# haoyu94/RoITr

Measured on AMD Instinct MI355X. Metric: point-cloud pairs/s, higher is better.
Workload: dtype f32; 1 GPU; 3DMatch-sized synthetic pairs: 5000 pts/cloud src+tgt, fp32, 3DMatch test settings (P=256 patches x 64 pts, 100 Sinkhorn iterations), full RIGA_v2 forward; n_points=5000, weights=closed-form, variant 'selective' (roitr_amd/weights.py); normals: field, cloud=uniform, correspondences_found=66241567

## Files before the change

include/roitr_engine.h:

```cpp
#ifndef ROITR_ENGINE_H
#define ROITR_ENGINE_H

#include <stddef.h>

#ifdef __cplusplus
extern "C" {
#endif

#ifndef ROITR_POINTOPS_H
typedef struct ihipStream_t* roitr_stream_t;
#endif

typedef struct RoitrGemm {
    int M, N, K;
    const float* A; const float* A2; int lda; const int* a_idx; int a_limit;
    const float* W; int ldw; const int* w_idx; int w_limit;
    const float* bias; float alpha; int relu;
    float* C; int ldc;
    int batch; long sA, sW, sC, sBias, sAidx, sWidx;
    const int* seg_off; int seg_a0, seg_w0;
    const float* ln_gamma; const float* ln_beta; const float* ln_res; const int* ln_res_idx; const float* ln_post;
    int ln_relu; float ln_eps;
    int bf16;
    const float* A_cat; int lda_cat; int k_cat;
// ... 177 lines not shown
int roitr_optimal_transport(const RoitrOT* a, roitr_stream_t stream);
int roitr_ot_stats(int enable, unsigned long long* out);

typedef struct RoitrFine {
    int pairs, num_corr, limit, k, mutual;
    float conf;
    const int* n_corr; const float* ot; const int* row_masks; const int* col_masks;
    const float* row_pts; const float* col_pts; const float* global_scores;
    unsigned char* flags; int* counts; int* offsets; int* n_out;
    float* out_row_pts; float* out_col_pts; float* out_scores; int* out_patch;
    long out_cap;
    const int* pair_off; int slots;
    int* pair_starts;
} RoitrFine;
int roitr_fine_matching(const RoitrFine* a, roitr_stream_t stream);

int roitr_build_padded_clouds(int pairs, int n_points, const float* pts, const int* pt_offset, const float* rot,
                              const float* trans, float* out_pts, int* out_offset, roitr_stream_t stream);
int roitr_node_occlusion_score(int n_nodes, int limit, const int* cloud_of_node, const int* pt_offset, const int* knn_idx,
                               const int* knn_mask, const int* node_masks, const float* d2_padded, float overlap_thres,
                               float* out, roitr_stream_t stream);
typedef struct RoitrNodeCorr {
    int pairs, limit, max_nodes;
    float pos_radius;
    const float* nodes; const int* node_offset; const int* node_masks;
    const float* points; const int* pt_offset; const int* knn_idx; const int* knn_mask;
    const float* rot; const float* trans;
    float* overlap; long mat_stride;
    int* out_idx; float* out_overlap; int* out_count;
    int n_nodes; float* nodes_t; float* radius;
// ... 73 lines not shown
```

roitr_amd/csrc/engine.cpp:

```cpp
#include <hip/hip_runtime.h>
#include <math.h>
#include <stdio.h>
#include <string.h>

#include <functional>
#include <map>
#include <string>
#include <vector>

#include "common.h"
#include "prof.h"
#include "roitr_engine.h"
#include "roitr_pointops.h"

extern "C" int roitr_build_pfold(int H, int heads, const float* wpe, const float* bpe, float* pfold, hipStream_t stream);

#define CHK(x)                    \
    do {                          \
        int s__ = (x);            \
        if (s__ != 0) return s__; \
    } while (0)

namespace {

// ... 1451 lines not shown
        c.tgt_corr = tgt_corr; c.src_corr = src_corr; c.corr_scores = cscore; c.n_corr = n_corr;
        c.xy = cxy; c.xy_stride = xystride; c.xy_ld = V.nmax[3];
        if (E.cfg.adaptive_coarse) CHK(roitr_adaptive_matching(&c, E.cfg.num_corr, 0.75f, st));
        else CHK(roitr_coarse_matching(&c, st));
    }
    if (compact) CHK(roitr_patch_offsets(B, n_corr, (int)NP, pair_off, st));
    const int* live_patches = compact ? pair_off + B : nullptr;
    {
        RoitrPatch pg; memset(&pg, 0, sizeof(pg));
        pg.pairs = B; pg.num_corr = P_; pg.limit = LIM; pg.n_corr = n_corr; pg.tgt_corr = tgt_corr; pg.src_corr = src_corr;
        pg.node_offset = D.off[3]; pg.pt_offset = D.off[0]; pg.knn_idx = kidx; pg.knn_mask = kmask; pg.points = pts_out;
        pg.tgt_rows = trows; pg.src_rows = srows; pg.tgt_masks = tmask; pg.src_masks = smask; pg.tgt_pts = tpts; pg.src_pts = spts;
        pg.pair_off = pair_off; pg.slots = compact ? (int)NP : 0;
        CHK(roitr_patch_gather(&pg, st));
    }
    {
        RoitrGemm g; memset(&g, 0, sizeof(g));
        g.M = LIM; g.N = LIM; g.K = C4; g.A = point_feats; g.lda = C4; g.a_idx = trows; g.a_limit = T1; g.W = point_feats; g.ldw = C4;
        g.w_idx = srows; g.w_limit = T1; g.alpha = 1.0f / sqrtf((float)C4); g.C = mscore; g.ldc = LIM; g.batch = (int)NP;
        g.sC = (long)LIM * LIM; g.sAidx = LIM; g.sWidx = LIM;
        g.batch_live = live_patches;
        if (E.cfg.operand_dtype == 1) {
            unsigned short* pf_h = A.get<unsigned short>((size_t)T1 * C4);
            if (A.fail) { roitr_set_error("arena exhausted (matching)", __FILE__, __LINE__); return ROITR_ERR_ARG; }
            RoitrGemm gh = g;
            gh.A = reinterpret_cast<const float*>(pf_h); gh.W = reinterpret_cast<const float*>(pf_h); gh.bf16 = ROITR_BF16_W | ROITR_BF16_A;
            if (roitr_gemm_bf16_supported(&gh)) {
                CHK(roitr_f32_to_bf16((long)T1 * C4, point_feats, pf_h, st));
                g = gh;
            }
        }
        CHK(roitr_gemm(&g, st));
    }
    {
        RoitrOT o; memset(&o, 0, sizeof(o));
        o.pairs = B; o.num_corr = P_; o.limit = LIM; o.num_iter = 100; o.n_corr = n_corr; o.scores = mscore; o.row_masks = tmask;
        o.col_masks = smask; o.alpha = E.ot_alpha; o.out = ot;
        o.pair_off = pair_off; o.slots = compact ? (int)NP : 0;
        CHK(roitr_optimal_transport(&o, st));
    }
    {
        RoitrFine fm; memset(&fm, 0, sizeof(fm));
        fm.pairs = B; fm.num_corr = P_; fm.limit = LIM; fm.k = E.cfg.fine_topk; fm.mutual = E.cfg.fine_mutual; fm.conf = E.cfg.fine_conf;
        fm.n_corr = n_corr; fm.ot = ot; fm.row_masks = tmask; fm.col_masks = smask; fm.row_pts = tpts; fm.col_pts = spts;
        fm.global_scores = E.cfg.fine_use_global_score ? cscore : nullptr;
        fm.flags = flags; fm.counts = counts; fm.offsets = offsets; fm.n_out = n_out;
        fm.out_row_pts = o_t; fm.out_col_pts = o_s; fm.out_scores = o_sc; fm.out_patch = io->out_patch; fm.out_cap = (long)cap;
        fm.pair_off = pair_off; fm.slots = compact ? (int)NP : 0; fm.pair_starts = io->pair_starts;
        CHK(roitr_fine_matching(&fm, st));
    }
    roitr_prof_end(ROITR_PROF_PH_MATCH, st);
    roitr_prof_end(ROITR_PROF_PH_FORWARD, st);
    return 0;
}


extern "C" int roitr_engine_forward_graph(void* h, const RoitrForwardIO* io, hipStream_t st)
{
    Engine& E = *(Engine*)h;
    if (!E.finalized) { roitr_set_error("engine not finalized", __FILE__, __LINE__); return ROITR_ERR_ARG; }
    if (!st || roitr_prof_is_enabled() || !E.taps.empty() || !E.injects.empty() || io->pairs <= 0) return roitr_engine_forward(h, io, st);
    std::vector<long> key;
    key.push_back(io->pairs);
// ... 73 lines not shown
```

roitr_amd/csrc/matching.hip:

```cpp
#include "common.h"
#include <cstdio>
#include <cstdlib>
#include "prof.h"
#include "roitr_engine.h"

namespace {

__device__ __forceinline__ float sq_norm3(float x, float y, float z)
{
#pragma clang fp contract(off)
    const float a = x * x, b = y * y, c = z * z;
    return (a + b) + c;
}
__device__ __forceinline__ float square_distance3(float sx, float sy, float sz, float s2, float tx, float ty, float tz, float t2)
{
#pragma clang fp contract(off)
    const float m = sx * tx;
    const float xy = __fmaf_rn(sz, tz, __fmaf_rn(sy, ty, m));
    const float a = -2.0f * xy;
    const float b = a + s2;
    return fmaxf(b + t2, 1e-12f);
}

__global__ __launch_bounds__(256) void p2n_assign_kernel(int n_points, const float* __restrict__ pts, const int* __restrict__ pt_offset,
// ... 381 lines not shown
    OT_TERM(s0, B, KARR, T_, 8); OT_TERM(s1, B, KARR, T_, 9); OT_TERM(s2, B, KARR, T_, 10); OT_TERM(s3, B, KARR, T_, 11);   \
    OT_TERM(s0, B, KARR, T_, 12); OT_TERM(s1, B, KARR, T_, 13); OT_TERM(s2, B, KARR, T_, 14); OT_TERM(s3, B, KARR, T_, 15)
__device__ __forceinline__ float ot_dot64(const float (&KARR)[64], float x, float init, int lane)
{
    const float x1 = __int_as_float(__builtin_amdgcn_ds_bpermute(((lane + 16) & 63) << 2, __float_as_int(x)));
    const float x2 = __int_as_float(__builtin_amdgcn_ds_bpermute(((lane + 32) & 63) << 2, __float_as_int(x)));
    const float x3 = __int_as_float(__builtin_amdgcn_ds_bpermute(((lane + 48) & 63) << 2, __float_as_int(x)));
    float s0 = init, s1 = 0.f, s2 = 0.f, s3 = 0.f;
    asm volatile("s_nop 1" : : "v"(x), "v"(s1), "v"(s2), "v"(s3));
    OT_BLOCK(x, KARR, 0);
    OT_BLOCK(x1, KARR, 1);
    OT_BLOCK(x2, KARR, 2);
    OT_BLOCK(x3, KARR, 3);
    return (s0 + s1) + (s2 + s3);
}
__global__ __launch_bounds__(64) void ot_kernel(RoitrOT a, unsigned long long* stats)
{
    __shared__ float T[64][65];
    __shared__ __attribute__((aligned(16))) float av[64];
    const int patch = blockIdx.x;
    const int lane = threadIdx.x;
    if (a.pair_off ? patch >= a.pair_off[a.pairs] : (patch % a.num_corr) >= a.n_corr[patch / a.num_corr]) return;
    float* out = a.out + (size_t)patch * OTN * OTN;
    const float alpha = *a.alpha;
    const float* sc = a.scores + (size_t)patch * 64 * 64;
    const bool rml = a.row_masks[(size_t)patch * 64 + lane] != 0, cml = a.col_masks[(size_t)patch * 64 + lane] != 0;
    const unsigned long long rbits = __ballot(rml), cbits = __ballot(cml);
    const int nvr = __popcll(rbits), nvc = __popcll(cbits);
    const float norm = -logf((float)nvr + (float)nvc);
#pragma unroll 8
    for (int i = 0; i < 64; ++i) T[i][lane] = sc[i * 64 + lane];
    __syncthreads();
    float KR[64], KC[64];
    float m = rml ? alpha : -1e6f;
    float lo = alpha;
#pragma unroll
    for (int j = 0; j < 64; ++j) {
        const bool ok = rml && ((cbits >> j) & 1);
        const float v = ok ? T[lane][j] : -1e6f;
        KR[j] = v;
        m = fmaxf(m, v);
        lo = ok ? fminf(lo, v) : lo;
    }
    if (__ballot(rml && m - lo > OT_FAST_SPREAD) != 0) {
        if (lane == 0) out[64 * OTN + 64] = __int_as_float(0x7fc00000);
        return;
    }
#pragma unroll
    for (int j = 0; j < 64; ++j) {
        KR[j] = (rml && ((cbits >> j) & 1)) ? expf(KR[j] - m) : 0.f;
        T[lane][j] = KR[j];
    }
    const float krd = rml ? expf(alpha - m) : 0.f;
    const float kdr = cml ? 1.0f : 0.f;
    const float kdd = 1.0f;
    __syncthreads();
    {
        const int R = lane >> 4, c = lane & 15;
#pragma unroll
        for (int t = 0; t < 4; ++t)
#pragma unroll
            for (int n = 0; n < 16; ++n) {
                const int e = ((R + t) & 3) * 16 + ((c - n) & 15);
                KR[t * 16 + n] = T[lane][e];
                KC[t * 16 + n] = T[e][lane];
            }
    }
    const float mu = rml ? expf(norm) : 0.f, nu = cml ? expf(norm) : 0.f;
    const float mu64 = expf(logf((float)nvc) + norm), nu64 = expf(logf((float)nvr) + norm);
    float al = 0.f, a64 = 0.f, bl = cml ? 1.0f : 0.f, b64 = 1.0f;
    for (int it = 0; it < a.num_iter; ++it) {
        const float rs = ot_dot64(KR, bl, krd * b64, lane);
        al = rml ? mu / rs : 0.f;
        a64 = mu64 / (wave_sum(kdr * bl) + kdd * b64);
        const float cs = ot_dot64(KC, al, kdr * a64, lane);
        const float bn = cml ? nu / cs : 0.f;
        const float b64n = nu64 / (wave_sum(krd * al) + kdd * a64);
        const bool same = __ballot(__float_as_int(bn) != __float_as_int(bl)) == 0 && __float_as_int(b64n) == __float_as_int(b64);
        bl = bn; b64 = b64n;
        if (same) { if (stats && lane == 0) atomicAdd(stats + 1, (unsigned long long)(a.num_iter - 1 - it)); break; }
    }
    if (stats && lane == 0) atomicAdd(stats, 1ull);
    {
        const bool bad = (rml && !(al > 0.f && al < INFINITY)) || (cml && !(bl > 0.f && bl < INFINITY)) || !(a64 > 0.f && a64 < INFINITY) ||
                         !(b64 > 0.f && b64 < INFINITY);
        if (__ballot(bad) != 0) {
            if (lane == 0) out[64 * OTN + 64] = __int_as_float(0x7fc00000);
            return;
        }
    }
    __syncthreads();
    const float ul = rml ? logf(al) - m : 0.f, vl = cml ? logf(bl) : 0.f;
    const float u64 = logf(a64) - alpha, v64 = logf(b64);
    av[lane] = ul;
    __syncthreads();
#pragma unroll 8
    for (int i = 0; i < 64; ++i) {
        const float sv = (cml && ((rbits >> i) & 1)) ? sc[i * 64 + lane] : -1e6f;
        out[i * OTN + lane] = sv + av[i] + vl - norm;
    }
    out[64 * OTN + lane] = (cml ? alpha : -1e6f) + u64 + vl - norm;
    out[lane * OTN + 64] = (rml ? alpha : -1e6f) + ul + v64 - norm;
    if (lane == 0) out[64 * OTN + 64] = alpha + u64 + v64 - norm;
}

#define OTL_ROT(X, N_) __int_as_float(__builtin_amdgcn_update_dpp(0, __float_as_int(X), 0x120 + (N_), 0xf, 0xf, false))
#define OTL_LOAD16(XA, SARR, VB, T_)                                                                                         \
    XA[(T_) * 16] = SARR[(T_) * 16] + VB;                                                                                     \
    XA[(T_) * 16 + 1] = SARR[(T_) * 16 + 1] + OTL_ROT(VB, 1);   XA[(T_) * 16 + 2] = SARR[(T_) * 16 + 2] + OTL_ROT(VB, 2);     \
    XA[(T_) * 16 + 3] = SARR[(T_) * 16 + 3] + OTL_ROT(VB, 3);   XA[(T_) * 16 + 4] = SARR[(T_) * 16 + 4] + OTL_ROT(VB, 4);     \
    XA[(T_) * 16 + 5] = SARR[(T_) * 16 + 5] + OTL_ROT(VB, 5);   XA[(T_) * 16 + 6] = SARR[(T_) * 16 + 6] + OTL_ROT(VB, 6);     \
    XA[(T_) * 16 + 7] = SARR[(T_) * 16 + 7] + OTL_ROT(VB, 7);   XA[(T_) * 16 + 8] = SARR[(T_) * 16 + 8] + OTL_ROT(VB, 8);     \
    XA[(T_) * 16 + 9] = SARR[(T_) * 16 + 9] + OTL_ROT(VB, 9);   XA[(T_) * 16 + 10] = SARR[(T_) * 16 + 10] + OTL_ROT(VB, 10); \
    XA[(T_) * 16 + 11] = SARR[(T_) * 16 + 11] + OTL_ROT(VB, 11); XA[(T_) * 16 + 12] = SARR[(T_) * 16 + 12] + OTL_ROT(VB, 12); \
    XA[(T_) * 16 + 13] = SARR[(T_) * 16 + 13] + OTL_ROT(VB, 13); XA[(T_) * 16 + 14] = SARR[(T_) * 16 + 14] + OTL_ROT(VB, 14); \
    XA[(T_) * 16 + 15] = SARR[(T_) * 16 + 15] + OTL_ROT(VB, 15)
__device__ __forceinline__ float ot_lse65(const float (&SARR)[64], float x, float extra, int lane)
{
// ... 9 lines not shown
#pragma unroll
    for (int i = 0; i < 64; ++i) mx = fmaxf(mx, X[i]);
    float s0 = __expf(extra - mx), s1 = 0.f, s2 = 0.f, s3 = 0.f;
#pragma unroll
    for (int i = 0; i < 64; i += 4) {
        s0 += __expf(X[i] - mx); s1 += __expf(X[i + 1] - mx); s2 += __expf(X[i + 2] - mx); s3 += __expf(X[i + 3] - mx);
    }
    return mx + __logf((s0 + s1) + (s2 + s3));
}
__device__ __forceinline__ float ot_lse_wave(float x, float extra)
{
    const float mx = fmaxf(wave_max(x), extra);
    return mx + __logf(wave_sum(__expf(x - mx)) + __expf(extra - mx));
}

__global__ __launch_bounds__(64) void ot_log_kernel(RoitrOT a, unsigned long long* stats)
{
    __shared__ float T[64][65];
    const int patch = blockIdx.x;
    const int lane = threadIdx.x;
    if (a.pair_off ? patch >= a.pair_off[a.pairs] : (patch % a.num_corr) >= a.n_corr[patch / a.num_corr]) return;
    float* out = a.out + (size_t)patch * OTN * OTN;
    {
        const float corner = out[64 * OTN + 64];
        if (corner == corner) return;
    }
    if (stats && lane == 0) atomicAdd(stats + 2, 1ull);
    const float alpha = *a.alpha;
    const float NINF = -1e6f;
    const float* sc = a.scores + (size_t)patch * 64 * 64;
    const bool rml = a.row_masks[(size_t)patch * 64 + lane] != 0, cml = a.col_masks[(size_t)patch * 64 + lane] != 0;
    const unsigned long long rbits = __ballot(rml), cbits = __ballot(cml);
    const int nvr = __popcll(rbits), nvc = __popcll(cbits);
    const float norm = -logf((float)nvr + (float)nvc);
#pragma unroll 8
    for (int i = 0; i < 64; ++i) T[i][lane] = (cml && ((rbits >> i) & 1)) ? sc[i * 64 + lane] : NINF;
// ... 23 lines not shown
        vl = vn;
    }
    __syncthreads();
    T[0][lane] = ul;
    __syncthreads();
#pragma unroll 8
    for (int i = 0; i < 64; ++i) {
        const float sv = (cml && ((rbits >> i) & 1)) ? sc[i * 64 + lane] : NINF;
        out[i * OTN + lane] = sv + T[0][i] + vl - norm;
    }
    out[64 * OTN + lane] = sdr + u64 + vl - norm;
    out[lane * OTN + 64] = srd + ul + v64 - norm;
    if (lane == 0) out[64 * OTN + 64] = alpha + u64 + v64 - norm;
}

__device__ __forceinline__ unsigned long long topk_mask(float v, int k, float conf)
{
    const int lane = threadIdx.x & 63;
    bool sel = false;
    for (int t = 0; t < k; ++t) {
        const float cand = sel ? -1.f : v;
        const float m = wave_max(cand);
        const unsigned long long eq = __ballot(cand == m);
        if (m >= 0.f && lane == __ffsll((long long)eq) - 1) sel = true;
    }
    return __ballot(sel && v > conf);
}

__global__ __launch_bounds__(256) void fine_flag_kernel(RoitrFine a)
{
    __shared__ float E[64][65];
    __shared__ unsigned long long rowm[64], colm[64];
    __shared__ int cnt_s[4];
    const int patch = blockIdx.x;
    const int tid = threadIdx.x, lane = tid & 63, wave = tid >> 6;
    const int L = a.limit;
    unsigned char* fl = a.flags + (size_t)patch * L * L;
    uint4* fl16 = reinterpret_cast<uint4*>(fl) + tid;
    if (a.pair_off ? patch >= a.pair_off[a.pairs] : (patch % a.num_corr) >= a.n_corr[patch / a.num_corr]) {
        if (tid == 0) a.counts[patch] = 0;
        return;
    }
    const float* sc = a.ot + (size_t)patch * (L + 1) * (L + 1);
    for (int e = tid; e < L * L; e += 256) { const int i = e >> 6, j = e & 63; E[i][j] = expf(sc[i * (L + 1) + j]); }
    __syncthreads();
    if (a.k <= 4) {
        if (wave < 2) {
            float bv[4] = {-1.f, -1.f, -1.f, -1.f};
            int bi[4] = {0, 0, 0, 0};
#pragma unroll 8
            for (int j = 0; j < 64; ++j) {
                float x = wave == 0 ? E[lane][j] : E[j][lane];
                int xi = j;
#pragma unroll
                for (int t = 0; t < 4; ++t) {
                    const bool up = x > bv[t];
                    const float tv = bv[t]; const int ti = bi[t];
                    bv[t] = up ? x : tv; bi[t] = up ? xi : ti;
                    x = up ? tv : x; xi = up ? ti : xi;
                }
            }
            unsigned long long m = 0ull;
#pragma unroll
            for (int t = 0; t < 4; ++t)
                if (t < a.k && bv[t] >= 0.f && bv[t] > a.conf) m |= 1ull << bi[t];
            if (wave == 0) rowm[lane] = m; else colm[lane] = m;
        }
    } else {
        for (int r = wave; r < 64; r += 4) {
            const unsigned long long mr = topk_mask(E[r][lane], a.k, a.conf);
            const unsigned long long mc = topk_mask(E[lane][r], a.k, a.conf);
            if (lane == 0) { rowm[r] = mr; colm[r] = mc; }
        }
    }
    __syncthreads();
    const int i = tid >> 2, j0 = (tid & 3) * 16;
    const int* cm = a.col_masks + (size_t)patch * L;
    const bool row_ok = a.row_masks[(size_t)patch * L + i] != 0;
    const unsigned long long rmask = rowm[i];
    unsigned w[4] = {0, 0, 0, 0};
    int local = 0;
#pragma unroll
    for (int jj = 0; jj < 16; ++jj) {
        const int j = j0 + jj;
        const bool rt = (rmask >> j) & 1, ct = (colm[j] >> i) & 1;
        const bool f = (a.mutual ? (rt && ct) : (rt || ct)) && row_ok && cm[j] != 0;
        w[jj >> 2] |= (f ? 1u : 0u) << (8 * (jj & 3));
        local += f ? 1 : 0;
    }
    *fl16 = make_uint4(w[0], w[1], w[2], w[3]);
    local = (int)wave_sum((float)local);
    if (lane == 0) cnt_s[wave] = local;
    __syncthreads();
    if (tid == 0) a.counts[patch] = cnt_s[0] + cnt_s[1] + cnt_s[2] + cnt_s[3];
}

__global__ __launch_bounds__(1024) void fine_scan_kernel(int n, const int* __restrict__ counts, int* __restrict__ offsets, int* __restrict__ n_out,
                                                         long out_cap, int pairs, int num_corr, const int* __restrict__ pair_off,
                                                         int* __restrict__ pair_starts)
{
    __shared__ int wsum[16];
    __shared__ int carry_s;
    const int tid = threadIdx.x, lane = tid & 63, wave = tid >> 6;
    if (tid == 0) carry_s = 0;
    __syncthreads();
    for (int base = 0; base < n; base += 1024) {
        const int i = base + tid;
        const int v = i < n ? counts[i] : 0;
        int incl = v;
// ... 52 lines not shown
    for (int u = 0; u < per; ++u) {
        const int e = tid * per + u;
        if (((fw[u >> 2] >> (8 * (u & 3))) & 1u) && pos < cap) {
            const int i = e / L, j = e % L;
            const float* rp = a.row_pts + ((size_t)patch * L + i) * 3;
            const float* cp = a.col_pts + ((size_t)patch * L + j) * 3;
            a.out_row_pts[(size_t)pos * 3] = rp[0]; a.out_row_pts[(size_t)pos * 3 + 1] = rp[1]; a.out_row_pts[(size_t)pos * 3 + 2] = rp[2];
            a.out_col_pts[(size_t)pos * 3] = cp[0]; a.out_col_pts[(size_t)pos * 3 + 1] = cp[1]; a.out_col_pts[(size_t)pos * 3 + 2] = cp[2];
            a.out_scores[pos] = expf(sc[i * (L + 1) + j]) * g;
            if (a.out_patch) a.out_patch[pos] = patch;
            ++pos;
        }
    }
}

}

extern "C" int roitr_point_to_node_partition(int b, int n_points, int n_nodes, const float* pts, const int* pt_offset,
                                             const float* nodes, const int* node_offset, const int* cloud_of_node, int limit,
                                             int* p2n, float* p2n_dist, int* node_masks, int* knn_idx, int* knn_mask, hipStream_t stream)
{
    if (n_points <= 0 || n_nodes <= 0) return ROITR_OK;
    ROITR_HIP(hipMemsetAsync(node_masks, 0, sizeof(int) * (size_t)n_nodes, stream));
    p2n_assign_kernel<<<div_up(n_points, 256), 256, 0, stream>>>(n_points, pts, pt_offset, nullptr, nodes, node_offset, b, p2n, p2n_dist, node_masks);
    ROITR_LAUNCH_CHECK();
    p2n_topk_kernel<<<n_nodes, 256, 0, stream>>>(pt_offset, node_offset, cloud_of_node, p2n, p2n_dist, limit, knn_idx, knn_mask);
    ROITR_LAUNCH_CHECK();
    return ROITR_OK;
}

// ... 115 lines not shown
    if (a->limit != 64) return ROITR_ERR_UNSUPPORTED;
    const int patches = a->pair_off ? a->slots : a->pairs * a->num_corr;
    if (patches <= 0) {
        ROITR_HIP(hipMemsetAsync(a->n_out, 0, sizeof(int), stream));
        if (a->pair_starts) ROITR_HIP(hipMemsetAsync(a->pair_starts, 0, sizeof(int) * ((size_t)a->pairs + 1), stream));
        return ROITR_OK;
    }
    fine_flag_kernel<<<patches, 256, 0, stream>>>(*a);
    ROITR_LAUNCH_CHECK();
    fine_scan_kernel<<<1, 1024, 0, stream>>>(patches, a->counts, a->offsets, a->n_out, a->out_cap, a->pairs, a->num_corr, a->pair_off, a->pair_starts);
    ROITR_LAUNCH_CHECK();
    fine_emit_kernel<<<patches, 256, 0, stream>>>(*a);
    ROITR_LAUNCH_CHECK();
    return ROITR_OK;
}
```

roitr_amd/ops.py:

```python
import torch

from . import _lib as L


def _i32c(t):
    return t.to(torch.int32).contiguous()


def calc_ppf(points, point_normals, ref_points, ref_normals, group_idx):
    m, k = group_idx.shape
    out = torch.empty((m, k, 4), dtype=torch.float32, device=points.device)
    grp = _i32c(group_idx)
    L.check(L.lib().roitr_calc_ppf(m, k, L.ptr(points.contiguous()), L.ptr(point_normals.contiguous()),
                                   L.ptr(ref_points.contiguous()), L.ptr(ref_normals.contiguous()), L.ptr(grp), L.ptr(out),
                                   L.stream_ptr()), "calc_ppf")
    return out


def calc_ppf_gpu(points, point_normals, patches, patch_normals):
    m, k, _ = patches.shape
    grp = torch.arange(m * k, dtype=torch.int32, device=points.device).view(m, k)
    return calc_ppf(points, point_normals, patches.reshape(-1, 3), patch_normals.reshape(-1, 3), grp)


# ... 90 lines not shown
    offs = torch.zeros(B, dtype=i32, device=dev)
    n_out = torch.zeros(1, dtype=i32, device=dev)
    o_r = torch.zeros((cap, 3), dtype=torch.float32, device=dev)
    o_c = torch.zeros((cap, 3), dtype=torch.float32, device=dev)
    o_s = torch.zeros(cap, dtype=torch.float32, device=dev)
    rm, cm = ref_knn_masks.to(i32).contiguous(), src_knn_masks.to(i32).contiguous()
    rp, cp = ref_knn_points.contiguous().float(), src_knn_points.contiguous().float()
    ms = matching_scores.contiguous().float()
    gs = global_scores.contiguous().float() if global_scores is not None else None
    a = _Fine(1, B, Lm, int(k), int(mutual), float(confidence_threshold), L.ptr(nc), L.ptr(ms), L.ptr(rm), L.ptr(cm), L.ptr(rp),
              L.ptr(cp), L.ptr(gs), L.ptr(flags), L.ptr(counts), L.ptr(offs), L.ptr(n_out), L.ptr(o_r), L.ptr(o_c), L.ptr(o_s), L.ptr(None), cap)
    L.check(L.lib().roitr_fine_matching(ctypes.byref(a), L.stream_ptr()), "fine_matching")
    n = int(n_out.item())
    return o_r[:n], o_c[:n], o_s[:n]


class _Gemm(ctypes.Structure):
    _fields_ = [("M", ctypes.c_int), ("N", ctypes.c_int), ("K", ctypes.c_int), ("A", _P), ("A2", _P), ("lda", ctypes.c_int),
                ("a_idx", _P), ("a_limit", ctypes.c_int), ("W", _P), ("ldw", ctypes.c_int), ("w_idx", _P), ("w_limit", ctypes.c_int),
                ("bias", _P), ("alpha", ctypes.c_float), ("relu", ctypes.c_int), ("C", _P), ("ldc", ctypes.c_int),
                ("batch", ctypes.c_int), ("sA", ctypes.c_long), ("sW", ctypes.c_long), ("sC", ctypes.c_long),
                ("sBias", ctypes.c_long), ("sAidx", ctypes.c_long), ("sWidx", ctypes.c_long), ("seg_off", _P),
                ("seg_a0", ctypes.c_int), ("seg_w0", ctypes.c_int),
                ("ln_gamma", _P), ("ln_beta", _P), ("ln_res", _P), ("ln_res_idx", _P), ("ln_post", _P),
                ("ln_relu", ctypes.c_int), ("ln_eps", ctypes.c_float), ("bf16", ctypes.c_int),
                ("A_cat", _P), ("lda_cat", ctypes.c_int), ("k_cat", ctypes.c_int),
                ("ip_feat", _P), ("ip_idx", _P), ("ip_dist2", _P), ("a_cat_idx", _P), ("batch_live", _P), ("w_piece", ctypes.c_long)]


BF16_W, BF16_A, BF16_C, BF16_X3 = 1, 2, 4, 8
# ... 269 lines not shown
```

Measured before the change: 6336 pairs/s.

## Fuse patch score GEMM, Sinkhorn OT and fine flagging into one kernel

For the fp32 operand path, a single patch_match kernel now computes each patch's 64x64 similarity tile, runs the exp-domain Sinkhorn solve and produces the fine top-k flags, all with the tile kept in shared memory. This avoids writing the score matrix out and reading it back across separate GEMM, OT and flag launches. Patches that fail the fast exp solve are appended to a declined list and handled afterwards by grid-stride log-domain OT and flag kernels. The cost is a heavier per-block kernel with one 64-thread wave per patch, plus an extra atomic-driven fallback path.

```diff
diff --git a/include/roitr_engine.h b/include/roitr_engine.h
--- a/include/roitr_engine.h
+++ b/include/roitr_engine.h
@@ -215,6 +215,7 @@
     int* pair_starts;
 } RoitrFine;
 int roitr_fine_matching(const RoitrFine* a, roitr_stream_t stream);
+int roitr_patch_match(const RoitrGemm* g, const RoitrOT* o, const RoitrFine* f, int* declined, roitr_stream_t stream);
 
 int roitr_build_padded_clouds(int pairs, int n_points, const float* pts, const int* pt_offset, const float* rot,
                               const float* trans, float* out_pts, int* out_offset, roitr_stream_t stream);
diff --git a/roitr_amd/csrc/engine.cpp b/roitr_amd/csrc/engine.cpp
--- a/roitr_amd/csrc/engine.cpp
+++ b/roitr_amd/csrc/engine.cpp
@@ -1489,39 +1489,37 @@
         pg.pair_off = pair_off; pg.slots = compact ? (int)NP : 0;
         CHK(roitr_patch_gather(&pg, st));
     }
-    {
-        RoitrGemm g; memset(&g, 0, sizeof(g));
-        g.M = LIM; g.N = LIM; g.K = C4; g.A = point_feats; g.lda = C4; g.a_idx = trows; g.a_limit = T1; g.W = point_feats; g.ldw = C4;
-        g.w_idx = srows; g.w_limit = T1; g.alpha = 1.0f / sqrtf((float)C4); g.C = mscore; g.ldc = LIM; g.batch = (int)NP;
-        g.sC = (long)LIM * LIM; g.sAidx = LIM; g.sWidx = LIM;
-        g.batch_live = live_patches;
-        if (E.cfg.operand_dtype == 1) {
-            unsigned short* pf_h = A.get<unsigned short>((size_t)T1 * C4);
-            if (A.fail) { roitr_set_error("arena exhausted (matching)", __FILE__, __LINE__); return ROITR_ERR_ARG; }
-            RoitrGemm gh = g;
-            gh.A = reinterpret_cast<const float*>(pf_h); gh.W = reinterpret_cast<const float*>(pf_h); gh.bf16 = ROITR_BF16_W | ROITR_BF16_A;
-            if (roitr_gemm_bf16_supported(&gh)) {
-                CHK(roitr_f32_to_bf16((long)T1 * C4, point_feats, pf_h, st));
-                g = gh;
-            }
+    RoitrGemm g; memset(&g, 0, sizeof(g));
+    g.M = LIM; g.N = LIM; g.K = C4; g.A = point_feats; g.lda = C4; g.a_idx = trows; g.a_limit = T1; g.W = point_feats; g.ldw = C4;
+    g.w_idx = srows; g.w_limit = T1; g.alpha = 1.0f / sqrtf((float)C4); g.C = mscore; g.ldc = LIM; g.batch = (int)NP;
+    g.sC = (long)LIM * LIM; g.sAidx = LIM; g.sWidx = LIM;
+    g.batch_live = live_patches;
+    RoitrOT o; memset(&o, 0, sizeof(o));
+    o.pairs = B; o.num_corr = P_; o.limit = LIM; o.num_iter = 100; o.n_corr = n_corr; o.scores = mscore; o.row_masks = tmask;
+    o.col_masks = smask; o.alpha = E.ot_alpha; o.out = ot;
+    o.pair_off = pair_off; o.slots = compact ? (int)NP : 0;
+    RoitrFine fm; memset(&fm, 0, sizeof(fm));
+    fm.pairs = B; fm.num_corr = P_; fm.limit = LIM; fm.k = E.cfg.fine_topk; fm.mutual = E.cfg.fine_mutual; fm.conf = E.cfg.fine_conf;
+    fm.n_corr = n_corr; fm.ot = ot; fm.row_masks = tmask; fm.col_masks = smask; fm.row_pts = tpts; fm.col_pts = spts;
+    fm.global_scores = E.cfg.fine_use_global_score ? cscore : nullptr;
+    fm.flags = flags; fm.counts = counts; fm.offsets = offsets; fm.n_out = n_out;
+    fm.out_row_pts = o_t; fm.out_col_pts = o_s; fm.out_scores = o_sc; fm.out_patch = io->out_patch; fm.out_cap = (long)cap;
+    fm.pair_off = pair_off; fm.slots = compact ? (int)NP : 0; fm.pair_starts = io->pair_starts;
+    if (E.cfg.operand_dtype != 1) {
+        int* declined = A.get<int>(NP + 1);
+        if (A.fail) { roitr_set_error("arena exhausted (matching)", __FILE__, __LINE__); return ROITR_ERR_ARG; }
+        CHK(roitr_patch_match(&g, &o, &fm, declined, st));
+    } else {
+        unsigned short* pf_h = A.get<unsigned short>((size_t)T1 * C4);
+        if (A.fail) { roitr_set_error("arena exhausted (matching)", __FILE__, __LINE__); return ROITR_ERR_ARG; }
+        RoitrGemm gh = g;
+        gh.A = reinterpret_cast<const float*>(pf_h); gh.W = reinterpret_cast<const float*>(pf_h); gh.bf16 = ROITR_BF16_W | ROITR_BF16_A;
+        if (roitr_gemm_bf16_supported(&gh)) {
+            CHK(roitr_f32_to_bf16((long)T1 * C4, point_feats, pf_h, st));
+            g = gh;
         }
         CHK(roitr_gemm(&g, st));
-    }
-    {
-        RoitrOT o; memset(&o, 0, sizeof(o));
-        o.pairs = B; o.num_corr = P_; o.limit = LIM; o.num_iter = 100; o.n_corr = n_corr; o.scores = mscore; o.row_masks = tmask;
-        o.col_masks = smask; o.alpha = E.ot_alpha; o.out = ot;
-        o.pair_off = pair_off; o.slots = compact ? (int)NP : 0;
         CHK(roitr_optimal_transport(&o, st));
-    }
-    {
-        RoitrFine fm; memset(&fm, 0, sizeof(fm));
-        fm.pairs = B; fm.num_corr = P_; fm.limit = LIM; fm.k = E.cfg.fine_topk; fm.mutual = E.cfg.fine_mutual; fm.conf = E.cfg.fine_conf;
-        fm.n_corr = n_corr; fm.ot = ot; fm.row_masks = tmask; fm.col_masks = smask; fm.row_pts = tpts; fm.col_pts = spts;
-        fm.global_scores = E.cfg.fine_use_global_score ? cscore : nullptr;
-        fm.flags = flags; fm.counts = counts; fm.offsets = offsets; fm.n_out = n_out;
-        fm.out_row_pts = o_t; fm.out_col_pts = o_s; fm.out_scores = o_sc; fm.out_patch = io->out_patch; fm.out_cap = (long)cap;
-        fm.pair_off = pair_off; fm.slots = compact ? (int)NP : 0; fm.pair_starts = io->pair_starts;
         CHK(roitr_fine_matching(&fm, st));
     }
     roitr_prof_end(ROITR_PROF_PH_MATCH, st);
diff --git a/roitr_amd/csrc/matching.hip b/roitr_amd/csrc/matching.hip
--- a/roitr_amd/csrc/matching.hip
+++ b/roitr_amd/csrc/matching.hip
@@ -419,13 +419,94 @@
     OT_BLOCK(x3, KARR, 3);
     return (s0 + s1) + (s2 + s3);
 }
+__device__ __forceinline__ bool ot_exp_solve(const float (*T)[65], float* m_s, int lane, bool rml, bool cml, unsigned long long rbits,
+                                             unsigned long long cbits, float alpha, float norm, int num_iter, unsigned long long* stats,
+                                             float& ul, float& vl, float& u64, float& v64)
+{
+    float KR[64], KC[64];
+    float m = rml ? alpha : -1e6f;
+    float lo = alpha;
+#pragma unroll
+    for (int j = 0; j < 64; ++j) {
+        const bool ok = rml && ((cbits >> j) & 1);
+        const float v = ok ? T[lane][j] : -1e6f;
+        m = fmaxf(m, v);
+        lo = ok ? fminf(lo, v) : lo;
+    }
+    if (__ballot(rml && m - lo > OT_FAST_SPREAD) != 0) return false;
+    m_s[lane] = m;
+    __syncthreads();
+    const float krd = rml ? expf(alpha - m) : 0.f;
+    const float kdr = cml ? 1.0f : 0.f;
+    const float kdd = 1.0f;
+    {
+        const int R = lane >> 4, c = lane & 15;
+#pragma unroll
+        for (int t = 0; t < 4; ++t)
+#pragma unroll
+            for (int n = 0; n < 16; ++n) {
+                const int e = ((R + t) & 3) * 16 + ((c - n) & 15);
+                KR[t * 16 + n] = (rml && ((cbits >> e) & 1)) ? expf(T[lane][e] - m) : 0.f;
+                KC[t * 16 + n] = (cml && ((rbits >> e) & 1)) ? expf(T[e][lane] - m_s[e]) : 0.f;
+            }
+    }
+    const int nvr = __popcll(rbits), nvc = __popcll(cbits);
+    const float mu = rml ? expf(norm) : 0.f, nu = cml ? expf(norm) : 0.f;
+    const float mu64 = expf(logf((float)nvc) + norm), nu64 = expf(logf((float)nvr) + norm);
+    float al = 0.f, a64 = 0.f, bl = cml ? 1.0f : 0.f, b64 = 1.0f;
+    for (int it = 0; it < num_iter; ++it) {
+        const float rs = ot_dot64(KR, bl, krd * b64, lane);
+        al = rml ? mu / rs : 0.f;
+        a64 = mu64 / (wave_sum(kdr * bl) + kdd * b64);
+        const float cs = ot_dot64(KC, al, kdr * a64, lane);
+        const float bn = cml ? nu / cs : 0.f;
+        const float b64n = nu64 / (wave_sum(krd * al) + kdd * a64);
+        const bool same = __ballot(__float_as_int(bn) != __float_as_int(bl)) == 0 && __float_as_int(b64n) == __float_as_int(b64);
+        bl = bn; b64 = b64n;
+        if (same) { if (stats && lane == 0) atomicAdd(stats + 1, (unsigned long long)(num_iter - 1 - it)); break; }
+    }
+    if (stats && lane == 0) atomicAdd(stats, 1ull);
+    {
+        const bool bad = (rml && !(al > 0.f && al < INFINITY)) || (cml && !(bl > 0.f && bl < INFINITY)) || !(a64 > 0.f && a64 < INFINITY) ||
+                         !(b64 > 0.f && b64 < INFINITY);
+        if (__ballot(bad) != 0) return false;
+    }
+    ul = rml ? logf(al) - m : 0.f; vl = cml ? logf(bl) : 0.f;
+    u64 = logf(a64) - alpha; v64 = logf(b64);
+    return true;
+}
+
+template <bool EXP>
+__device__ __forceinline__ void ot_exp_output(float (*T)[65], float* av, float* __restrict__ out, int lane, bool rml, bool cml,
+                                              unsigned long long rbits, float alpha, float norm, float ul, float vl, float u64, float v64)
+{
+    __syncthreads();
+    av[lane] = ul;
+    __syncthreads();
+#pragma unroll 8
+    for (int i = 0; i < 64; ++i) {
+        const float sv = (cml && ((rbits >> i) & 1)) ? T[i][lane] : -1e6f;
+        const float o = sv + av[i] + vl - norm;
+        out[i * OTN + lane] = o;
+        if (EXP) T[i][lane] = expf(o);
+    }
+    out[64 * OTN + lane] = (cml ? alpha : -1e6f) + u64 + vl - norm;
+    out[lane * OTN + 64] = (rml ? alpha : -1e6f) + ul + v64 - norm;
+    if (lane == 0) out[64 * OTN + 64] = alpha + u64 + v64 - norm;
+}
+
+__device__ __forceinline__ bool ot_patch_live(const RoitrOT& a, int patch)
+{
+    return a.pair_off ? patch < a.pair_off[a.pairs] : (patch % a.num_corr) < a.n_corr[patch / a.num_corr];
+}
+
 __global__ __launch_bounds__(64) void ot_kernel(RoitrOT a, unsigned long long* stats)
 {
     __shared__ float T[64][65];
-    __shared__ __attribute__((aligned(16))) float av[64];
+    __shared__ float m_s[64], av[64];
     const int patch = blockIdx.x;
     const int lane = threadIdx.x;
-    if (a.pair_off ? patch >= a.pair_off[a.pairs] : (patch % a.num_corr) >= a.n_corr[patch / a.num_corr]) return;
+    if (!ot_patch_live(a, patch)) return;
     float* out = a.out + (size_t)patch * OTN * OTN;
     const float alpha = *a.alpha;
     const float* sc = a.scores + (size_t)patch * 64 * 64;
@@ -436,77 +517,12 @@
 #pragma unroll 8
     for (int i = 0; i < 64; ++i) T[i][lane] = sc[i * 64 + lane];
     __syncthreads();
-    float KR[64], KC[64];
-    float m = rml ? alpha : -1e6f;
-    float lo = alpha;
-#pragma unroll
-    for (int j = 0; j < 64; ++j) {
-        const bool ok = rml && ((cbits >> j) & 1);
-        const float v = ok ? T[lane][j] : -1e6f;
-        KR[j] = v;
-        m = fmaxf(m, v);
-        lo = ok ? fminf(lo, v) : lo;
-    }
-    if (__ballot(rml && m - lo > OT_FAST_SPREAD) != 0) {
+    float ul, vl, u64, v64;
+    if (!ot_exp_solve(T, m_s, lane, rml, cml, rbits, cbits, alpha, norm, a.num_iter, stats, ul, vl, u64, v64)) {
         if (lane == 0) out[64 * OTN + 64] = __int_as_float(0x7fc00000);
         return;
     }
-#pragma unroll
-    for (int j = 0; j < 64; ++j) {
-        KR[j] = (rml && ((cbits >> j) & 1)) ? expf(KR[j] - m) : 0.f;
-        T[lane][j] = KR[j];
-    }
-    const float krd = rml ? expf(alpha - m) : 0.f;
-    const float kdr = cml ? 1.0f : 0.f;
-    const float kdd = 1.0f;
-    __syncthreads();
-    {
-        const int R = lane >> 4, c = lane & 15;
-#pragma unroll
-        for (int t = 0; t < 4; ++t)
-#pragma unroll
-            for (int n = 0; n < 16; ++n) {
-                const int e = ((R + t) & 3) * 16 + ((c - n) & 15);
-                KR[t * 16 + n] = T[lane][e];
-                KC[t * 16 + n] = T[e][lane];
-            }
-    }
-    const float mu = rml ? expf(norm) : 0.f, nu = cml ? expf(norm) : 0.f;
-    const float mu64 = expf(logf((float)nvc) + norm), nu64 = expf(logf((float)nvr) + norm);
-    float al = 0.f, a64 = 0.f, bl = cml ? 1.0f : 0.f, b64 = 1.0f;
-    for (int it = 0; it < a.num_iter; ++it) {
-        const float rs = ot_dot64(KR, bl, krd * b64, lane);
-        al = rml ? mu / rs : 0.f;
-        a64 = mu64 / (wave_sum(kdr * bl) + kdd * b64);
-        const float cs = ot_dot64(KC, al, kdr * a64, lane);
-        const float bn = cml ? nu / cs : 0.f;
-        const float b64n = nu64 / (wave_sum(krd * al) + kdd * a64);
-        const bool same = __ballot(__float_as_int(bn) != __float_as_int(bl)) == 0 && __float_as_int(b64n) == __float_as_int(b64);
-        bl = bn; b64 = b64n;
-        if (same) { if (stats && lane == 0) atomicAdd(stats + 1, (unsigned long long)(a.num_iter - 1 - it)); break; }
-    }
-    if (stats && lane == 0) atomicAdd(stats, 1ull);
-    {
-        const bool bad = (rml && !(al > 0.f && al < INFINITY)) || (cml && !(bl > 0.f && bl < INFINITY)) || !(a64 > 0.f && a64 < INFINITY) ||
-                         !(b64 > 0.f && b64 < INFINITY);
-        if (__ballot(bad) != 0) {
-            if (lane == 0) out[64 * OTN + 64] = __int_as_float(0x7fc00000);
-            return;
-        }
-    }
-    __syncthreads();
-    const float ul = rml ? logf(al) - m : 0.f, vl = cml ? logf(bl) : 0.f;
-    const float u64 = logf(a64) - alpha, v64 = logf(b64);
-    av[lane] = ul;
-    __syncthreads();
-#pragma unroll 8
-    for (int i = 0; i < 64; ++i) {
-        const float sv = (cml && ((rbits >> i) & 1)) ? sc[i * 64 + lane] : -1e6f;
-        out[i * OTN + lane] = sv + av[i] + vl - norm;
-    }
-    out[64 * OTN + lane] = (cml ? alpha : -1e6f) + u64 + vl - norm;
-    out[lane * OTN + 64] = (rml ? alpha : -1e6f) + ul + v64 - norm;
-    if (lane == 0) out[64 * OTN + 64] = alpha + u64 + v64 - norm;
+    ot_exp_output<false>(T, av, out, lane, rml, cml, rbits, alpha, norm, ul, vl, u64, v64);
 }
 
 #define OTL_ROT(X, N_) __int_as_float(__builtin_amdgcn_update_dpp(0, __float_as_int(X), 0x120 + (N_), 0xf, 0xf, false))
@@ -546,12 +562,10 @@
     return mx + __logf(wave_sum(__expf(x - mx)) + __expf(extra - mx));
 }
 
-__global__ __launch_bounds__(64) void ot_log_kernel(RoitrOT a, unsigned long long* stats)
-{
-    __shared__ float T[64][65];
-    const int patch = blockIdx.x;
+__device__ __forceinline__ void ot_log_patch(const RoitrOT& a, int patch, unsigned long long* stats, float (*T)[65])
+{
     const int lane = threadIdx.x;
-    if (a.pair_off ? patch >= a.pair_off[a.pairs] : (patch % a.num_corr) >= a.n_corr[patch / a.num_corr]) return;
+    if (!ot_patch_live(a, patch)) return;
     float* out = a.out + (size_t)patch * OTN * OTN;
     {
         const float corner = out[64 * OTN + 64];
@@ -605,6 +619,12 @@
     if (lane == 0) out[64 * OTN + 64] = alpha + u64 + v64 - norm;
 }
 
+__global__ __launch_bounds__(64) void ot_log_kernel(RoitrOT a, unsigned long long* stats)
+{
+    __shared__ float T[64][65];
+    ot_log_patch(a, blockIdx.x, stats, T);
+}
+
 __device__ __forceinline__ unsigned long long topk_mask(float v, int k, float conf)
 {
     const int lane = threadIdx.x & 63;
@@ -618,57 +638,35 @@
     return __ballot(sel && v > conf);
 }
 
-__global__ __launch_bounds__(256) void fine_flag_kernel(RoitrFine a)
-{
-    __shared__ float E[64][65];
-    __shared__ unsigned long long rowm[64], colm[64];
-    __shared__ int cnt_s[4];
-    const int patch = blockIdx.x;
-    const int tid = threadIdx.x, lane = tid & 63, wave = tid >> 6;
+__device__ __forceinline__ unsigned long long fine_topk4(const float (*E)[65], int lane, bool col, int k, float conf)
+{
+    float bv[4] = {-1.f, -1.f, -1.f, -1.f};
+    int bi[4] = {0, 0, 0, 0};
+#pragma unroll 8
+    for (int j = 0; j < 64; ++j) {
+        float x = col ? E[j][lane] : E[lane][j];
+        int xi = j;
+#pragma unroll
+        for (int t = 0; t < 4; ++t) {
+            const bool up = x > bv[t];
+            const float tv = bv[t]; const int ti = bi[t];
+            bv[t] = up ? x : tv; bi[t] = up ? xi : ti;
+            x = up ? tv : x; xi = up ? ti : xi;
+        }
+    }
+    unsigned long long m = 0ull;
+#pragma unroll
+    for (int t = 0; t < 4; ++t)
+        if (t < k && bv[t] >= 0.f && bv[t] > conf) m |= 1ull << bi[t];
+    return m;
+}
+
+__device__ __forceinline__ uint4 fine_flag16(const RoitrFine& a, int patch, int i, int j0, unsigned long long rmask,
+                                             const unsigned long long* colm, int& count)
+{
     const int L = a.limit;
-    unsigned char* fl = a.flags + (size_t)patch * L * L;
-    uint4* fl16 = reinterpret_cast<uint4*>(fl) + tid;
-    if (a.pair_off ? patch >= a.pair_off[a.pairs] : (patch % a.num_corr) >= a.n_corr[patch / a.num_corr]) {
-        if (tid == 0) a.counts[patch] = 0;
-        return;
-    }
-    const float* sc = a.ot + (size_t)patch * (L + 1) * (L + 1);
-    for (int e = tid; e < L * L; e += 256) { const int i = e >> 6, j = e & 63; E[i][j] = expf(sc[i * (L + 1) + j]); }
-    __syncthreads();
-    if (a.k <= 4) {
-        if (wave < 2) {
-            float bv[4] = {-1.f, -1.f, -1.f, -1.f};
-            int bi[4] = {0, 0, 0, 0};
-#pragma unroll 8
-            for (int j = 0; j < 64; ++j) {
-                float x = wave == 0 ? E[lane][j] : E[j][lane];
-                int xi = j;
-#pragma unroll
-                for (int t = 0; t < 4; ++t) {
-                    const bool up = x > bv[t];
-                    const float tv = bv[t]; const int ti = bi[t];
-                    bv[t] = up ? x : tv; bi[t] = up ? xi : ti;
-                    x = up ? tv : x; xi = up ? ti : xi;
-                }
-            }
-            unsigned long long m = 0ull;
-#pragma unroll
-            for (int t = 0; t < 4; ++t)
-                if (t < a.k && bv[t] >= 0.f && bv[t] > a.conf) m |= 1ull << bi[t];
-            if (wave == 0) rowm[lane] = m; else colm[lane] = m;
-        }
-    } else {
-        for (int r = wave; r < 64; r += 4) {
-            const unsigned long long mr = topk_mask(E[r][lane], a.k, a.conf);
-            const unsigned long long mc = topk_mask(E[lane][r], a.k, a.conf);
-            if (lane == 0) { rowm[r] = mr; colm[r] = mc; }
-        }
-    }
-    __syncthreads();
-    const int i = tid >> 2, j0 = (tid & 3) * 16;
     const int* cm = a.col_masks + (size_t)patch * L;
     const bool row_ok = a.row_masks[(size_t)patch * L + i] != 0;
-    const unsigned long long rmask = rowm[i];
     unsigned w[4] = {0, 0, 0, 0};
     int local = 0;
 #pragma unroll
@@ -679,11 +677,57 @@
         w[jj >> 2] |= (f ? 1u : 0u) << (8 * (jj & 3));
         local += f ? 1 : 0;
     }
-    *fl16 = make_uint4(w[0], w[1], w[2], w[3]);
+    count = local;
+    return make_uint4(w[0], w[1], w[2], w[3]);
+}
+
+__device__ __forceinline__ bool fine_patch_live(const RoitrFine& a, int patch)
+{
+    return a.pair_off ? patch < a.pair_off[a.pairs] : (patch % a.num_corr) < a.n_corr[patch / a.num_corr];
+}
+
+__device__ __forceinline__ void fine_flag_patch(const RoitrFine& a, int patch, float (*E)[65], unsigned long long* rowm, unsigned long long* colm,
+                                                int* cnt_s)
+{
+    const int tid = threadIdx.x, lane = tid & 63, wave = tid >> 6;
+    const int L = a.limit;
+    unsigned char* fl = a.flags + (size_t)patch * L * L;
+    uint4* fl16 = reinterpret_cast<uint4*>(fl) + tid;
+    if (!fine_patch_live(a, patch)) {
+        if (tid == 0) a.counts[patch] = 0;
+        return;
+    }
+    const float* sc = a.ot + (size_t)patch * (L + 1) * (L + 1);
+    for (int e = tid; e < L * L; e += 256) { const int i = e >> 6, j = e & 63; E[i][j] = expf(sc[i * (L + 1) + j]); }
+    __syncthreads();
+    if (a.k <= 4) {
+        if (wave < 2) {
+            const unsigned long long m = fine_topk4(E, lane, wave == 1, a.k, a.conf);
+            if (wave == 0) rowm[lane] = m; else colm[lane] = m;
+        }
+    } else {
+        for (int r = wave; r < 64; r += 4) {
+            const unsigned long long mr = topk_mask(E[r][lane], a.k, a.conf);
+            const unsigned long long mc = topk_mask(E[lane][r], a.k, a.conf);
+            if (lane == 0) { rowm[r] = mr; colm[r] = mc; }
+        }
+    }
+    __syncthreads();
+    const int i = tid >> 2, j0 = (tid & 3) * 16;
+    int local = 0;
+    *fl16 = fine_flag16(a, patch, i, j0, rowm[i], colm, local);
     local = (int)wave_sum((float)local);
     if (lane == 0) cnt_s[wave] = local;
     __syncthreads();
     if (tid == 0) a.counts[patch] = cnt_s[0] + cnt_s[1] + cnt_s[2] + cnt_s[3];
+}
+
+__global__ __launch_bounds__(256) void fine_flag_kernel(RoitrFine a)
+{
+    __shared__ float E[64][65];
+    __shared__ unsigned long long rowm[64], colm[64];
+    __shared__ int cnt_s[4];
+    fine_flag_patch(a, blockIdx.x, E, rowm, colm, cnt_s);
 }
 
 __global__ __launch_bounds__(1024) void fine_scan_kernel(int n, const int* __restrict__ counts, int* __restrict__ offsets, int* __restrict__ n_out,
@@ -766,6 +810,166 @@
     }
 }
 
+typedef float pm_f32x16 __attribute__((ext_vector_type(16)));
+constexpr int PM_MAX_K = 2048, PM_LDR = 12, PM_BOFF = 2 * 64 * PM_LDR;
+__device__ __attribute__((aligned(16))) float pm_zero_row[PM_MAX_K];
+constexpr int PM_LIST_GRID = 1024;
+
+__global__ __launch_bounds__(64) void patch_match_kernel(RoitrGemm g, RoitrOT a, RoitrFine f, int* __restrict__ declined,
+                                                         unsigned long long* stats, int n)
+{
+    __shared__ __attribute__((aligned(16))) float T[64][65];
+    __shared__ float m_s[64], av[64];
+    __shared__ unsigned long long rowm[64], colm[64];
+    const int patch = xcd_block_id_live(n);
+    if (patch < 0) return;
+    const int lane = threadIdx.x;
+    if (!ot_patch_live(a, patch)) {
+        if (lane == 0) f.counts[patch] = 0;
+        return;
+    }
+    {
+        const int p = lane & 1, r0 = lane >> 1;
+        const int* ai = g.a_idx ? g.a_idx + (size_t)patch * g.sAidx : nullptr;
+        const int* wi = g.w_idx ? g.w_idx + (size_t)patch * g.sWidx : nullptr;
+        const float* A = g.A + (size_t)patch * g.sA;
+        const float* W = g.W + (size_t)patch * g.sW;
+        const float* ar[2]; const float* wr[2];
+#pragma unroll
+        for (int j = 0; j < 2; ++j) {
+            const int r = r0 + 32 * j;
+            const int sa = ai ? ai[r] : r, sw = wi ? wi[r] : r;
+            ar[j] = (sa >= 0 && (g.a_limit <= 0 || sa < g.a_limit)) ? A + (size_t)sa * g.lda : pm_zero_row;
+            wr[j] = (sw >= 0 && (g.w_limit <= 0 || sw < g.w_limit)) ? W + (size_t)sw * g.ldw : pm_zero_row;
+        }
+        float4 pa[2][2], pb[2][2];
+        auto fetch = [&](int hs) {
+            const int off = (hs >> 1) * 32 + 4 * (2 * (hs & 1) + p);
+#pragma unroll
+            for (int j = 0; j < 2; ++j) {
+                pa[j][0] = *reinterpret_cast<const float4*>(ar[j] + off); pa[j][1] = *reinterpret_cast<const float4*>(ar[j] + off + 16);
+                pb[j][0] = *reinterpret_cast<const float4*>(wr[j] + off); pb[j][1] = *reinterpret_cast<const float4*>(wr[j] + off + 16);
+            }
+        };
+        pm_f32x16 acc[2][2];
+#pragma unroll
+        for (int x = 0; x < 2; ++x)
+#pragma unroll
+            for (int y = 0; y < 2; ++y)
+#pragma unroll
+                for (int i = 0; i < 16; ++i) acc[x][y][i] = 0.f;
+        float* Ls = &T[0][0];
+        const int kh = lane >> 5, ml = lane & 31;
+        const int nh = g.K / 16;
+        fetch(0);
+        for (int hs = 0; hs < nh; ++hs) {
+            __syncthreads();
+#pragma unroll
+            for (int j = 0; j < 2; ++j) {
+                const int r = r0 + 32 * j;
+                *reinterpret_cast<float4*>(Ls + r * PM_LDR + 4 * p) = make_float4(pa[j][0].x, pa[j][0].z, pa[j][1].x, pa[j][1].z);
+                *reinterpret_cast<float4*>(Ls + (64 + r) * PM_LDR + 4 * p) = make_float4(pa[j][0].y, pa[j][0].w, pa[j][1].y, pa[j][1].w);
+                *reinterpret_cast<float4*>(Ls + PM_BOFF + r * PM_LDR + 4 * p) = make_float4(pb[j][0].x, pb[j][0].z, pb[j][1].x, pb[j][1].z);
+                *reinterpret_cast<float4*>(Ls + PM_BOFF + (64 + r) * PM_LDR + 4 * p) = make_float4(pb[j][0].y, pb[j][0].w, pb[j][1].y, pb[j][1].w);
+            }
+            __syncthreads();
+            if (hs + 1 < nh) fetch(hs + 1);
+            float4 af[2][2], bf[2][2];
+#pragma unroll
+            for (int x = 0; x < 2; ++x)
+#pragma unroll
+                for (int q = 0; q < 2; ++q) {
+                    af[x][q] = *reinterpret_cast<const float4*>(Ls + (kh * 64 + x * 32 + ml) * PM_LDR + 4 * q);
+                    bf[x][q] = *reinterpret_cast<const float4*>(Ls + PM_BOFF + (kh * 64 + x * 32 + ml) * PM_LDR + 4 * q);
+                }
+            __builtin_amdgcn_sched_barrier(0);
+#pragma unroll
+            for (int q = 0; q < 2; ++q)
+#pragma unroll
+                for (int c = 0; c < 4; ++c)
+#pragma unroll
+                    for (int x = 0; x < 2; ++x)
+#pragma unroll
+                        for (int y = 0; y < 2; ++y) {
+                            const float av_ = c == 0 ? af[x][q].x : c == 1 ? af[x][q].y : c == 2 ? af[x][q].z : af[x][q].w;
+                            const float bv_ = c == 0 ? bf[y][q].x : c == 1 ? bf[y][q].y : c == 2 ? bf[y][q].z : bf[y][q].w;
+                            acc[x][y] = __builtin_amdgcn_mfma_f32_32x32x2f32(av_, bv_, acc[x][y], 0, 0, 0);
+                        }
+            __builtin_amdgcn_sched_barrier(0);
+        }
+        __syncthreads();
+        const float bv = 0.f;
+#pragma unroll
+        for (int x = 0; x < 2; ++x)
+#pragma unroll
+            for (int y = 0; y < 2; ++y)
+#pragma unroll
+                for (int i = 0; i < 16; ++i) T[x * 32 + (i & 3) + 8 * (i >> 2) + 4 * kh][y * 32 + ml] = acc[x][y][i] * g.alpha + bv;
+        __syncthreads();
+    }
+    float* out = a.out + (size_t)patch * OTN * OTN;
+    const float alpha = *a.alpha;
+    const bool rml = a.row_masks[(size_t)patch * 64 + lane] != 0, cml = a.col_masks[(size_t)patch * 64 + lane] != 0;
+    const unsigned long long rbits = __ballot(rml), cbits = __ballot(cml);
+    const float norm = -logf((float)__popcll(rbits) + (float)__popcll(cbits));
+    float ul, vl, u64, v64;
+    if (!ot_exp_solve(T, m_s, lane, rml, cml, rbits, cbits, alpha, norm, a.num_iter, stats, ul, vl, u64, v64)) {
+        float* sc = g.C + (size_t)patch * g.sC;
+#pragma unroll 8
+        for (int i = 0; i < 64; ++i) sc[(size_t)i * g.ldc + lane] = T[i][lane];
+        if (lane == 0) {
+            out[64 * OTN + 64] = __int_as_float(0x7fc00000);
+            declined[1 + atomicAdd(declined, 1)] = patch;
+        }
+        return;
+    }
+    ot_exp_output<true>(T, av, out, lane, rml, cml, rbits, alpha, norm, ul, vl, u64, v64);
+    __syncthreads();
+    if (f.k <= 4) {
+        rowm[lane] = fine_topk4(T, lane, false, f.k, f.conf);
+        colm[lane] = fine_topk4(T, lane, true, f.k, f.conf);
+    } else {
+        for (int r = 0; r < 64; ++r) {
+            const unsigned long long mr = topk_mask(T[r][lane], f.k, f.conf);
+            const unsigned long long mc = topk_mask(T[lane][r], f.k, f.conf);
+            if (lane == 0) { rowm[r] = mr; colm[r] = mc; }
+        }
+    }
+    __syncthreads();
+    uint4* fl16 = reinterpret_cast<uint4*>(f.flags + (size_t)patch * 64 * 64);
+    int total = 0;
+#pragma unroll
+    for (int q = 0; q < 4; ++q) {
+        const int t = q * 64 + lane, i = t >> 2;
+        int c = 0;
+        fl16[t] = fine_flag16(f, patch, i, (t & 3) * 16, rowm[i], colm, c);
+        total += c;
+    }
+    total = (int)wave_sum((float)total);
+    if (lane == 0) f.counts[patch] = total;
+}
+
+__global__ __launch_bounds__(64) void ot_log_list_kernel(RoitrOT a, const int* __restrict__ declined, unsigned long long* stats)
+{
+    __shared__ float T[64][65];
+    const int n = declined[0];
+    for (int e = blockIdx.x; e < n; e += gridDim.x) {
+        __syncthreads();
+        ot_log_patch(a, declined[1 + e], stats, T);
+    }
+}
+__global__ __launch_bounds__(256) void fine_flag_list_kernel(RoitrFine a, const int* __restrict__ declined)
+{
+    __shared__ float E[64][65];
+    __shared__ unsigned long long rowm[64], colm[64];
+    __shared__ int cnt_s[4];
+    const int n = declined[0];
+    for (int e = blockIdx.x; e < n; e += gridDim.x) {
+        __syncthreads();
+        fine_flag_patch(a, declined[1 + e], E, rowm, colm, cnt_s);
+    }
+}
+
 }
 
 extern "C" int roitr_point_to_node_partition(int b, int n_points, int n_nodes, const float* pts, const int* pt_offset,
@@ -911,3 +1115,32 @@
     ROITR_LAUNCH_CHECK();
     return ROITR_OK;
 }
+
+extern "C" int roitr_patch_match(const RoitrGemm* g, const RoitrOT* o, const RoitrFine* f, int* declined, hipStream_t stream)
+{
+    if (o->pairs <= 0) return roitr_fine_matching(f, stream);
+    const int patches = o->pair_off ? o->slots : o->pairs * o->num_corr;
+    auto al16 = [](const void* p) { return ((uintptr_t)p & 15) == 0; };
+    if (o->limit != 64 || f->limit != 64 || g->M != 64 || g->N != 64 || g->batch != patches || g->K <= 0 || g->K % 32 || g->K > PM_MAX_K ||
+        g->lda % 4 || g->ldw % 4 || g->sA % 4 || g->sW % 4 || !al16(g->A) || !al16(g->W) || g->bf16 || g->A2 || g->bias || g->relu || g->ln_gamma ||
+        g->seg_off || g->A_cat || g->ip_feat || g->ldc != 64 || g->sC != 64 * 64 || g->C != o->scores || f->ot != o->out || f->pairs != o->pairs ||
+        f->num_corr != o->num_corr || f->pair_off != o->pair_off || f->slots != o->slots || f->n_corr != o->n_corr ||
+        f->row_masks != o->row_masks || f->col_masks != o->col_masks || !declined)
+        return ROITR_ERR_UNSUPPORTED;
+    if (patches <= 0) return roitr_fine_matching(f, stream);
+    const double bytes = 2.0 * 64 * g->K * 4.0 + 2.0 * 64 * 4 + 65.0 * 65 * 4 + 64.0 * 64 + 4, flops = 2.0 * 64 * 64 * g->K;
+    if (o->pair_off) roitr_prof_begin_live(ROITR_PROF_OT, bytes, flops, o->pair_off + o->pairs, stream);
+    else roitr_prof_begin2(ROITR_PROF_OT, (double)patches * bytes, (double)patches * flops, stream);
+    unsigned long long* sd = ot_stats().for_current_device();
+    ROITR_HIP(hipMemsetAsync(declined, 0, sizeof(int), stream));
+    patch_match_kernel<<<xcd_grid(patches), 64, 0, stream>>>(*g, *o, *f, declined, sd, patches);
+    ot_log_list_kernel<<<PM_LIST_GRID, 64, 0, stream>>>(*o, declined, sd);
+    fine_flag_list_kernel<<<PM_LIST_GRID, 256, 0, stream>>>(*f, declined);
+    roitr_prof_end(ROITR_PROF_OT, stream);
+    ROITR_LAUNCH_CHECK();
+    fine_scan_kernel<<<1, 1024, 0, stream>>>(patches, f->counts, f->offsets, f->n_out, f->out_cap, f->pairs, f->num_corr, f->pair_off, f->pair_starts);
+    ROITR_LAUNCH_CHECK();
+    fine_emit_kernel<<<patches, 256, 0, stream>>>(*f);
+    ROITR_LAUNCH_CHECK();
+    return ROITR_OK;
+}
diff --git a/roitr_amd/ops.py b/roitr_amd/ops.py
--- a/roitr_amd/ops.py
+++ b/roitr_amd/ops.py
@@ -128,6 +128,72 @@
     n = int(n_out.item())
     return o_r[:n], o_c[:n], o_s[:n]
 
+
+def matching_tail(feats, tgt_rows, src_rows, row_masks, col_masks, row_pts, col_pts, alpha, k, mutual=True,
+                  confidence_threshold=0.05, n_corr=None, num_corr=None, pair_off=None, global_scores=None, num_iter=100, fused=True, graph=False):
+    dev = feats.device
+    i32 = torch.int32
+    S, Lm = tgt_rows.shape
+    C = feats.shape[1]
+    compact = pair_off is not None
+    pairs = (pair_off.numel() - 1) if compact else n_corr.numel()
+    if not compact:
+        num_corr = int(num_corr) if num_corr is not None else S // pairs
+        assert pairs * num_corr == S
+    cap = S * Lm * int(k) * (1 if mutual else 2)
+    fe = feats.contiguous().float()
+    tr, sr = _i32c(tgt_rows), _i32c(src_rows)
+    rm, cm = _i32c(row_masks), _i32c(col_masks)
+    rp, cp = row_pts.contiguous().float(), col_pts.contiguous().float()
+    po = _i32c(pair_off) if compact else None
+    nc = _i32c(n_corr) if n_corr is not None else torch.zeros(pairs, dtype=i32, device=dev)
+    gs = global_scores.contiguous().float() if global_scores is not None else None
+    al = torch.as_tensor(alpha, dtype=torch.float32, device=dev).reshape(1).contiguous()
+    z = lambda *shape, dt=torch.float32: torch.zeros(shape, dtype=dt, device=dev)
+    r = dict(scores=z(S, Lm, Lm), ot=z(S, Lm + 1, Lm + 1), flags=z(S * Lm * Lm, dt=torch.uint8), counts=z(S, dt=i32), offsets=z(S, dt=i32),
+             n_out=z(1, dt=i32), row_pts=z(cap, 3), col_pts=z(cap, 3), scores_out=z(cap), patch_out=z(cap, dt=i32), pair_starts=z(pairs + 1, dt=i32))
+    live = L.ptr(po[pairs:]) if compact else None
+    g = _Gemm(Lm, Lm, C, L.ptr(fe), L.ptr(None), C, L.ptr(tr), fe.shape[0], L.ptr(fe), C, L.ptr(sr), fe.shape[0], L.ptr(None),
+              1.0 / float(C) ** 0.5, 0, L.ptr(r["scores"]), Lm, S, 0, 0, Lm * Lm, 0, Lm, Lm, L.ptr(None), 0, 0)
+    g.alpha = float(1.0 / torch.sqrt(torch.tensor(float(C), dtype=torch.float32)))
+    g.batch_live = live
+    slots = S if compact else 0
+    o = _OT(pairs, num_corr or 0, Lm, int(num_iter), L.ptr(nc), L.ptr(r["scores"]), L.ptr(rm), L.ptr(cm), L.ptr(al), L.ptr(r["ot"]),
+            L.ptr(po), slots)
+    f = _Fine(pairs, num_corr or 0, Lm, int(k), int(mutual), float(confidence_threshold), L.ptr(nc), L.ptr(r["ot"]), L.ptr(rm), L.ptr(cm),
+              L.ptr(rp), L.ptr(cp), L.ptr(gs), L.ptr(r["flags"]), L.ptr(r["counts"]), L.ptr(r["offsets"]), L.ptr(r["n_out"]),
+              L.ptr(r["row_pts"]), L.ptr(r["col_pts"]), L.ptr(r["scores_out"]), L.ptr(r["patch_out"]), cap, L.ptr(po), slots,
+              L.ptr(r["pair_starts"]))
+    lib = L.lib()
+    declined = z(S + 1, dt=i32)
+
+    def launch():
+        if fused:
+            L.check(lib.roitr_patch_match(ctypes.byref(g), ctypes.byref(o), ctypes.byref(f), L.ptr(declined), L.stream_ptr()), "patch_match")
+        else:
+            L.check(lib.roitr_gemm(ctypes.byref(g), L.stream_ptr()), "gemm")
+            L.check(lib.roitr_optimal_transport(ctypes.byref(o), L.stream_ptr()), "optimal_transport")
+            L.check(lib.roitr_fine_matching(ctypes.byref(f), L.stream_ptr()), "fine_matching")
+
+    if graph:
+        torch.cuda.synchronize(dev)
+        cg = torch.cuda.CUDAGraph()
+        with torch.cuda.graph(cg):
+            launch()
+        torch.cuda.synchronize(dev)
+        for t in r.values():
+            t.zero_()
+        cg.replay()
+    else:
+        launch()
+    torch.cuda.synchronize(dev)
+    return r
+
+
+def ot_stats(enable):
+    out = (ctypes.c_ulonglong * 3)()
+    L.check(L.lib().roitr_ot_stats(ctypes.c_int(enable), out), "ot_stats")
+    return tuple(int(v) for v in out)
 
 class _Gemm(ctypes.Structure):
     _fields_ = [("M", ctypes.c_int), ("N", ctypes.c_int), ("K", ctypes.c_int), ("A", _P), ("A2", _P), ("lda", ctypes.c_int),
```

New measurement: 6336 pairs/s, median of 3. About the same (+0.0%).
